# anuunchin/learned-quantization

Hardware: AMD Instinct MI355X
Metric: images/sec training with fake-quant layer, CIFAR-10 bs=256, 1/2/4/8 MI355X (higher is better)
Workload: dtype f32; 1 GPU; fake-quant fwd+bwd (split) on conv-activation batch 256x3x224x224 fp32 per GPU, per_channel scales, lambda=1e-11; per_gpu_batch=256, global_batch=256, parallelism=dp1, buffer_sets=4, launch=eager

## Files before the change

learned_quantization_amd/csrc/lq_kernels.hip:

```cpp
#include <hip/hip_runtime.h>
#include <hip/hip_ext.h>
#include <stdarg.h>
#include <stdlib.h>
#include <stdint.h>
#include <stdio.h>
#include <string.h>

#include <new>
#include <algorithm>
#include <vector>

#include "lq_hip.h"

#include "lq_batch.hpp"
#include "lq_stream2.hpp"
#include "lq_pack.hpp"

namespace lq {

enum Mode { MODE_ROW_BIG = 0, MODE_ROW_SMALL = 1, MODE_COL = 2 };

constexpr int64_t kColRbFused = 48;
constexpr int64_t kColRbBwd = 128;

// ... 519 lines not shown
#undef LQ_PIPE
        return check_hip("pipelined column launch") ? -1 : 1;
        }
    }
    if constexpr (OP == OP_FWD) {
        return 0;
    } else {
        bool seg = false;
        if (pl.L >= 5 && pl.L <= 64 && pl.L % 4 != 0) {
            const int nw = (int)(pl.L + 6) / 4;
            int tl = 1;
            while ((1 << tl) < nw) ++tl;
            const double eff = (double)nw / (double)(1 << tl);
            seg = eff < (OP == OP_FUSED ? 0.8 : 0.7);
        }
        if (!(off & 16384) && seg && pl.R < 4294967296ll) {
            constexpr int kSegU = 2;
            const int rpb = (kBlock * kSegU * 4 - 3) / (int)pl.L;
            const int64_t blocks = ceil_div(pl.R, (int64_t)rpb);
            if (blocks <= 2147483647ll) {
                const FastDiv fL = make_fastdiv((uint32_t)pl.L), fG = make_fastdiv((uint32_t)p.G);
                if (nt) hipLaunchKernelGGL((k_row_seg<OP, 1, kSegU>), dim3((unsigned)blocks), dim3(kBlock), 0, st, p, fL, fG, pl.R, (int)pl.L, rpb, n);
                else hipLaunchKernelGGL((k_row_seg<OP, 0, kSegU>), dim3((unsigned)blocks), dim3(kBlock), 0, st, p, fL, fG, pl.R, (int)pl.L, rpb, n);
                return check_hip("row-segment launch") ? -1 : 1;
            }
        }
        LQ_KNOB(win_all, "LQ_TUNE_WIN", 1);
        if (!(off & 128) && pl.L >= 5 && pl.R < 4294967296ll && (pl.L % 4 != 0 || (win_all && pl.L > 64))) {
            const int nwin = (int)(pl.L % 4 ? (pl.L + 3 + 3) / 4 : pl.L / 4);
            int lg = 1;
            while ((1 << lg) < nwin && lg < 6) ++lg;
            int V = lg == 6 ? (nwin + 63) / 64 : 1;
            if constexpr (OP == OP_BWD) {
                if (nwin >= 17 && nwin <= 32) { lg = 4; V = 2; }
                else if (nwin >= 33 && nwin <= 48) { lg = 4; V = 3; }
                else if (nwin >= 49 && nwin <= 55) { lg = 5; V = 2; }
                else if (nwin >= 65 && nwin <= 84) { lg = 5; V = 3; }
            } else {
                if (nwin >= 17 && nwin <= 32 && (nwin <= 19 || pl.L % 16 == 0)) { lg = 4; V = 2; }
                else if (nwin >= 33 && nwin <= 64) { lg = 5; V = 2; }
            }
            const int U = V == 1 ? 2 : 1;
            const int64_t rows_per_block = (int64_t)kWavesPerBlock * (64 >> lg) * U;
            const int64_t blocks = ceil_div(pl.R, rows_per_block);
            if (blocks <= 2147483647ll && V <= 5) {
                const FastDiv fG = make_fastdiv((uint32_t)p.G);
#define LQ_WIN(NT_, LG_, V_, U_) hipLaunchKernelGGL((k_row_win<OP, NT_, LG_, V_, U_>), dim3((unsigned)blocks), dim3(kBlock), 0, st, p, fG, pl.R, (int)pl.L, n)
#define LQ_WIN2(NT_) do { \
                switch (lg * 8 + V) { \
                    case 1 * 8 + 1: LQ_WIN(NT_, 1, 1, 2); break; \
                    case 2 * 8 + 1: LQ_WIN(NT_, 2, 1, 2); break; \
                    case 3 * 8 + 1: LQ_WIN(NT_, 3, 1, 2); break; \
                    case 4 * 8 + 1: LQ_WIN(NT_, 4, 1, 2); break; \
                    case 4 * 8 + 2: LQ_WIN(NT_, 4, 2, 1); break; \
                    case 4 * 8 + 3: if constexpr (OP == OP_BWD || kDevKnobs) LQ_WIN(NT_, 4, 3, 1); break; \
                    case 5 * 8 + 1: if constexpr (OP != OP_BWD || kDevKnobs) LQ_WIN(NT_, 5, 1, 2); break; \
                    case 5 * 8 + 2: LQ_WIN(NT_, 5, 2, 1); break; \
                    case 5 * 8 + 3: if constexpr (OP == OP_BWD || kDevKnobs) LQ_WIN(NT_, 5, 3, 1); break; \
                    case 6 * 8 + 1: if constexpr (OP == OP_BWD || kDevKnobs) LQ_WIN(NT_, 6, 1, 2); break; \
                    case 6 * 8 + 2: LQ_WIN(NT_, 6, 2, 1); break; \
                    case 6 * 8 + 3: LQ_WIN(NT_, 6, 3, 1); break; \
                    case 6 * 8 + 4: LQ_WIN(NT_, 6, 4, 1); break; \
                    default: LQ_WIN(NT_, 6, 5, 1); break; \
                } } while (0)
#ifdef LQ_DEV_KNOBS
                LQ_KNOB(geom, "LQ_TUNE_WIN_GEOM", 0);
                if (geom >= 100 && nt && ((geom / 10) % 10) * (1 << (geom / 100)) >= nwin) {
                    const int glg = geom / 100, gu = geom % 10;
                    const int64_t gblocks = ceil_div(pl.R, (int64_t)kWavesPerBlock * (64 >> glg) * gu);
                    bool done = true;
#define LQ_WING(LG_, V_, U_) hipLaunchKernelGGL((k_row_win<OP, 1, LG_, V_, U_>), dim3((unsigned)gblocks), dim3(kBlock), 0, st, p, fG, pl.R, (int)pl.L, n)
                    switch (geom) {
                        case 421: LQ_WING(4, 2, 1); break;
                        case 422: LQ_WING(4, 2, 2); break;
                        case 431: LQ_WING(4, 3, 1); break;
                        case 432: LQ_WING(4, 3, 2); break;
                        case 521: LQ_WING(5, 2, 1); break;
                        case 522: LQ_WING(5, 2, 2); break;
                        case 531: LQ_WING(5, 3, 1); break;
                        case 532: LQ_WING(5, 3, 2); break;
                        case 541: LQ_WING(5, 4, 1); break;
                        case 414: LQ_WING(4, 1, 4); break;
                        case 514: LQ_WING(5, 1, 4); break;
                        default: done = false;
                    }
#undef LQ_WING
                    if (done) return check_hip("row-window launch") ? -1 : 1;
                }
#endif
                if (nt) LQ_WIN2(1); else LQ_WIN2(0);
#undef LQ_WIN2
#undef LQ_WIN
                return check_hip("row-window launch") ? -1 : 1;
            }
        }
        if ((off & 8) || pl.L > 64 || pl.L < 8 || pl.L % 4 != 0) return 0;
        const int lg = row_small_lpr_log2_vec(pl.L);
        LQ_KNOB(tiny_u, "LQ_TUNE_TINY_U", 2);
        int U = (1 << lg) < tiny_u ? (1 << lg) : tiny_u;
        if (U != 2 && U != 4) U = 2;
        const int64_t rows_per_block = (int64_t)kWavesPerBlock * (64 >> lg) * U;
        const int64_t blocks = ceil_div(pl.R, rows_per_block);
        if (blocks > 2147483647ll) return 0;
        if (pl.R >= 4294967296ll) return 0;
        const int gm = (p.outer == 1) ? 0 : 1;
#define LQ_TINY3(NT_, U_, LG_) do { \
            if (gm == 0) hipLaunchKernelGGL((k_row_tiny<OP, NT_, U_, LG_, 0>), dim3((unsigned)blocks), dim3(kBlock), 0, st, p, pl.R, (int)pl.L); \
            else hipLaunchKernelGGL((k_row_tiny<OP, NT_, U_, LG_, 1>), dim3((unsigned)blocks), dim3(kBlock), 0, st, p, pl.R, (int)pl.L); } while (0)
#ifdef LQ_DEV_KNOBS
#define LQ_TINY2(NT_) do { \
            if (lg == 1) LQ_TINY3(NT_, 2, 1); \
            else if (lg == 2) { if (U == 2) LQ_TINY3(NT_, 2, 2); else LQ_TINY3(NT_, 4, 2); } \
            else if (lg == 3) { if (U == 2) LQ_TINY3(NT_, 2, 3); else LQ_TINY3(NT_, 4, 3); } \
            else { if (U == 2) LQ_TINY3(NT_, 2, 4); else LQ_TINY3(NT_, 4, 4); } } while (0)
#else
#define LQ_TINY2(NT_) do { \
            if (lg == 1) LQ_TINY3(NT_, 2, 1); \
            else if (lg == 2) LQ_TINY3(NT_, 2, 2); \
            else if (lg == 3) LQ_TINY3(NT_, 2, 3); \
            else LQ_TINY3(NT_, 2, 4); } while (0)
#endif
        if (nt) LQ_TINY2(1); else LQ_TINY2(0);
#undef LQ_TINY2
#undef LQ_TINY3
        return check_hip("tiny-row launch") ? -1 : 1;
    }
}

template <int OP>
constexpr bool kStreamOp = OP == OP_FWD || OP == OP_BWD || OP == OP_FUSED;

template <int OP>
static int launch_traverse(Plan& pl, const Params& p, hipStream_t st) {
    using O = OpT<OP>;
    if (!kStreamOp<OP> && pl.mode == MODE_ROW_BIG && pl.bs != kBlock) return fail(LQ_EINVAL, "internal: operation %d planned with %d-thread units", OP, pl.bs);
    {
        const int r2 = launch_stream2<OP>(pl, p, st);
        if (r2 < 0) return LQ_EHIP;
        if (r2 > 0) return LQ_OK;
    }
    if (pl.mode == MODE_ROW_BIG) {
        const bool vec = aligned(p.P, 16) && (!O::kDy || aligned(p.dy, 16)) && (!O::kStore || aligned(p.out, 16));
        LQ_KNOB(tune_chunk, "LQ_TUNE_CHUNK", 1);
        LQ_KNOB(forced_bs, "LQ_TUNE_BS", 0);
        if (pl.bs == 512 && vec && tune_chunk && !p.direct && !forced_bs && pl.np_ws >= pl.R * row_chunks(pl.L, 1024)) {
            auto fill = [&](int64_t CH) { return (double)pl.L / (double)(row_chunks(pl.L, CH) * CH); };
            const bool k2_form = (OP == OP_BWD || (OP == OP_FUSED && p.tmode >= 1)) && (double)pl.R * (double)pl.L * 4.0 >= (double)kNtBytes;
            const bool small = k2_form ? (row_chunks(pl.L, 4096) > 1 && fill(1024) > fill(4096) + 0.1) : (fill(1024) > fill(2048) + 0.05);
            if (small) {
                pl.bs = 256;
                pl.CH = 1024;
                pl.nc = row_chunks(pl.L, 1024);
                pl.np = pl.R * pl.nc;
                pl.gstride = pl.nc;
                pl.stride1 = p.G * pl.nc;
                pl.n2 = pl.nc;
            }
        }
        const int64_t units = pl.R * pl.nc;
        if (units > 2147483647ll) return fail(LQ_EINVAL, "too many work units (%lld)", (long long)units);
        const int64_t outer_f = pl.R / p.G;
        const int grid3d = (p.G <= 65535 && outer_f <= 65535 && pl.R == outer_f * p.G) ? 1 : 0;
        const dim3 grid = grid3d ? dim3((unsigned)pl.nc, (unsigned)p.G, (unsigned)outer_f) : dim3((unsigned)units);
        const bool nt = kStreamOp<OP> && vec && (double)pl.R * (double)pl.L * 4.0 >= (double)kNtBytes;
        LQ_KNOB(tune_u2, "LQ_TUNE_U2", -1);
        const bool want_u2 = tune_u2 >= 0 ? tune_u2 == 1 : (OP == OP_BWD || p.tmode >= 1);
        const bool u2 = (OP == OP_BWD || OP == OP_FUSED) && want_u2 && vec && nt && pl.bs == 512;
        auto needs_tail = [&](int64_t CH) {
            const int64_t r = pl.L % CH;
            return pl.L % 4 != 0 || (pl.L > CH && r != 0 && r * 8 <= CH);
        };
        if constexpr (OP == OP_BWD || OP == OP_FUSED) if (u2) {
            const int64_t nc2 = row_chunks(pl.L, (int64_t)pl.bs * 8);
            const dim3 grid2 = grid3d ? dim3((unsigned)nc2, (unsigned)p.G, (unsigned)outer_f) : dim3((unsigned)(pl.R * nc2));
            int64_t keep_from = OP == OP_BWD ? mall_keep_from(pl.R * pl.L) : 0;
#ifdef LQ_DEV_KNOBS
            if (g_dev_flags_host & 0x1000) keep_from = -1 - keep_from;
#endif
            if (needs_tail((int64_t)pl.bs * 8))
                hipExtLaunchKernelGGL((k_row_stream<OP, 4, 512, 1, 2, 1>), grid2, dim3(512), 0, st, g_prof_start, g_prof_stop, 0, p, pl.L, nc2, grid3d, keep_from);
            else
                hipExtLaunchKernelGGL((k_row_stream<OP, 4, 512, 1, 2, 0>), grid2, dim3(512), 0, st, g_prof_start, g_prof_stop, 0, p, pl.L, nc2, grid3d, keep_from);
            pl.CH = pl.bs * 8;
            pl.nc = nc2;
            pl.np = pl.R * nc2;
            pl.gstride = nc2;
            pl.stride1 = p.G * nc2;
            pl.n2 = nc2;
            return check_hip("traversal launch");
        }
        const bool tail1 = needs_tail((int64_t)pl.CH);
#define LQ_LAUNCH_STREAM(VEC_, BS_, NT_) do { \
        constexpr bool kTail0 = kDevKnobs || (VEC_ == 4 && !(OP == OP_FWD && (BS_ != kBlock || NT_ != 0)) && !(OP == OP_BWD && BS_ == 512 && NT_ == 1)); \
        constexpr bool kTail1 = kDevKnobs || !(OP == OP_BWD && VEC_ == 4 && BS_ == 512 && NT_ == 1); \
        if (VEC_ == 1 || tail1) { if constexpr (kTail1) hipExtLaunchKernelGGL((k_row_stream<OP, VEC_, BS_, NT_, 1, 1>), grid, dim3(BS_), 0, st, g_prof_start, g_prof_stop, 0, p, pl.L, pl.nc, grid3d, (int64_t)0); } \
        else { if constexpr (kTail0) hipExtLaunchKernelGGL((k_row_stream<OP, VEC_, BS_, NT_, 1, 0>), grid, dim3(BS_), 0, st, g_prof_start, g_prof_stop, 0, p, pl.L, pl.nc, grid3d, (int64_t)0); } } while (0)
        if constexpr (!kStreamOp<OP>) {
            if (vec) LQ_LAUNCH_STREAM(4, 256, 0);
            else LQ_LAUNCH_STREAM(1, 256, 0);
        } else if (!kDevKnobs && OP == OP_FWD && vec && !tail1 && (pl.bs != kBlock || nt)) {
            return fail(LQ_EINVAL, "internal: streaming-size forward of aligned rows reached the row stream");
        } else if (!kDevKnobs && OP == OP_BWD && vec && nt && pl.bs == 512) {
            return fail(LQ_EINVAL, "internal: streaming-size scale gradient reached the one-float4 row stream");
        } else if (vec) {
#ifdef LQ_DEV_KNOBS
            if (pl.bs == 1024) {
                if (nt) LQ_LAUNCH_STREAM(4, 1024, 1);
                else LQ_LAUNCH_STREAM(4, 1024, 0);
            } else
#endif
            if (pl.bs == 512) {
                if (nt) LQ_LAUNCH_STREAM(4, 512, 1);
                else LQ_LAUNCH_STREAM(4, 512, 0);
            } else {
                if (nt) LQ_LAUNCH_STREAM(4, 256, 1);
                else LQ_LAUNCH_STREAM(4, 256, 0);
            }
        } else {
#ifdef LQ_DEV_KNOBS
            if (pl.bs == 1024) LQ_LAUNCH_STREAM(1, 1024, 0);
            else
#endif
            if (pl.bs == 512) LQ_LAUNCH_STREAM(1, 512, 0);
            else LQ_LAUNCH_STREAM(1, 256, 0);
        }
#undef LQ_LAUNCH_STREAM
    } else if (pl.mode == MODE_ROW_SMALL) {
        const bool vec = row_small_vec(pl, p.P, O::kDy ? p.dy : nullptr, O::kStore ? p.out : nullptr);
        const int lg = vec ? row_small_lpr_log2_vec(pl.L) : pl.lpr_log2;
        const int64_t blocks = ceil_div(pl.R, kBlock >> lg);
        if (blocks > 2147483647ll) return fail(LQ_EINVAL, "too many blocks (%lld)", (long long)blocks);
        if (vec) hipLaunchKernelGGL((k_row_small<OP, 4>), dim3((unsigned)blocks), dim3(kBlock), 0, st, p, pl.R, (int)pl.L, lg);
        else hipLaunchKernelGGL((k_row_small<OP, 1>), dim3((unsigned)blocks), dim3(kBlock), 0, st, p, pl.R, (int)pl.L, lg);
    } else {
        int variant;
        int64_t nbx;
        col_variant(pl, p.P, O::kDy ? p.dy : nullptr, O::kStore ? p.out : nullptr, variant, nbx);
        const int64_t blocks = nbx * pl.ysplit;
        if (blocks > 2147483647ll) return fail(LQ_EINVAL, "too many blocks (%lld)", (long long)blocks);
        hipLaunchKernelGGL((k_col<OP>), dim3((unsigned)blocks), dim3(kBlock), 0, st, p, pl.C, pl.rps, nbx, variant, pl.ysplit);
    }
    return check_hip("traversal launch");
}

static bool finalize_cols_single(const FinGeom& f) {
    return finalize_cols_ok(f.groups, f.gstride, f.n1, f.stride1, f.n2) && f.n1 <= 64 && f.n1 * f.groups * f.n2 >= 131072;
}

template <int OP, bool COLS = true>
static int launch_finalize(const Params& p, FinGeom f, hipStream_t st) {
    const int form = finalize_form(f.groups, f.n1, f.stride1, f.n2);
    if (COLS && finalize_cols_single(f)) {
        if constexpr (COLS) hipLaunchKernelGGL((k_finalize_cols<OP>), dim3((unsigned)ceil_div(f.groups, 64 / f.n2)), dim3(kBlock), 0, st, p, f);
    } else if (form == 0) {
        hipLaunchKernelGGL((k_finalize_thread<OP>), dim3((unsigned)ceil_div(f.groups, kBlock)), dim3(kBlock), 0, st, p, f);
    } else if (form == 1) {
        hipLaunchKernelGGL((k_finalize_block<OP, 64>), dim3((unsigned)f.groups), dim3(64), 0, st, p, f);
    } else if (form == 2) {
        hipLaunchKernelGGL((k_finalize_block<OP, 256>), dim3((unsigned)f.groups), dim3(256), 0, st, p, f);
    } else {
        hipLaunchKernelGGL((k_finalize_block<OP, 1024>), dim3((unsigned)f.groups), dim3(1024), 0, st, p, f);
    }
    return check_hip("finalize launch");
}

static FinGeom group_geom(const Plan& pl, int64_t outer, int64_t G, int64_t inner) {
    FinGeom f;
    memset(&f, 0, sizeof(f));
    f.groups = G;
    f.gstride = pl.gstride;
    f.n1 = pl.n1;
    f.stride1 = pl.stride1;
    f.n2 = pl.n2;
    f.count = (double)outer * (double)inner;
    return f;
}

static FinGeom global_geom(const Plan& pl, int64_t outer, int64_t G, int64_t inner) {
    FinGeom f;
    memset(&f, 0, sizeof(f));
    f.groups = 1;
    f.gstride = 0;
    f.n1 = 1;
    f.stride1 = 0;
    f.n2 = pl.np;
    f.count = (double)outer * (double)G * (double)inner;
    return f;
}

static Params base_params(const float* P, const float* s, int64_t outer, int64_t G, int64_t inner) {
    Params p;
    memset(&p, 0, sizeof(p));
    p.P = P;
    p.s = s;
    p.outer = outer;
    p.G = G;
    p.inner = inner;
    return p;
}

static bool make_conv_tile(ConvTile& ct, int64_t hw, int64_t ci, int64_t co, int64_t outer, int64_t G, int64_t inner);
static int64_t conv_tile_partials(const ConvTile& ct, int64_t G);
static void conv_tile_fin(const ConvTile& ct, int64_t G, int64_t& gstride, int64_t& n1, int64_t& stride1, int64_t& n2);

}

using namespace lq;

#define LQ_REQUIRE_PTR(x)                                                      \
    do {                                                                       \
        if (!(x)) return fail(LQ_EINVAL, "%s: argument '%s' is NULL", __func__, #x); \
        if (!aligned((x), 4)) return fail(LQ_EALIGN, "%s: argument '%s' is not 4-byte aligned", __func__, #x); \
    } while (0)

extern "C" {

int lq_version(void) { return LQ_ABI_VERSION; }

#ifdef LQ_DEV_KNOBS
int lq_dev_set_ablate(int mask) {
    return hipMemcpyToSymbol(HIP_SYMBOL(lq::g_ablate), &mask, sizeof(int)) == hipSuccess ? LQ_OK : LQ_EHIP;
}
#endif

#ifdef LQ_DEV_KNOBS
int lq_dev_set_flags(int bits) {
    g_dev_flags_host = bits;
    return hipMemcpyToSymbol(HIP_SYMBOL(lq::g_dev_flags), &bits, sizeof(int)) == hipSuccess ? LQ_OK : LQ_EHIP;
}
#endif

#ifdef LQ_DEV_KNOBS
int lq_dev_set_trace(void* buf) {
    unsigned long long* b = (unsigned long long*)buf;
    return hipMemcpyToSymbol(HIP_SYMBOL(lq::g_trace), &b, sizeof(b)) == hipSuccess ? LQ_OK : LQ_EHIP;
}
#endif

int lq_profile_events(void* start, void* stop) {
    g_prof_start = (hipEvent_t)start;
    g_prof_stop = (hipEvent_t)stop;
    return LQ_OK;
}

const char* lq_last_error(void) { return g_err; }

const char* lq_status_string(int status) {
    switch (status) {
        case LQ_OK: return "LQ_OK";
        case LQ_EINVAL: return "LQ_EINVAL";
        case LQ_EHIP: return "LQ_EHIP";
        case LQ_EWORKSPACE: return "LQ_EWORKSPACE";
        case LQ_EALIGN: return "LQ_EALIGN";
        default: return "LQ_UNKNOWN";
    }
}

size_t lq_workspace_bytes(int64_t outer, int64_t G, int64_t inner) {
    if (outer <= 0 || G <= 0 || inner <= 0) return 0;
    return ws_bytes_for(make_plan(outer, G, inner));
}

int lq_fq_forward(const float* P, const float* s, float* out, void* q, int q_dtype, int64_t outer, int64_t G,
                  int64_t inner, void* stream) {
    int rc = check_desc(outer, G, inner);
    if (rc) return rc;
    LQ_REQUIRE_PTR(P);
    LQ_REQUIRE_PTR(s);
    if (!out && !q) return fail(LQ_EINVAL, "lq_fq_forward: both out and q are NULL");
    if (q_dtype < LQ_Q_NONE || q_dtype > LQ_Q_I8) return fail(LQ_EINVAL, "lq_fq_forward: bad q_dtype %d", q_dtype);
    if ((q != nullptr) != (q_dtype != LQ_Q_NONE)) return fail(LQ_EINVAL, "lq_fq_forward: q and q_dtype disagree");
    Plan pl = make_plan(outer, G, inner);
    Params p = base_params(P, s, outer, G, inner);
    p.q = q;
    p.q_dtype = q_dtype;
    if (out) {
        if (!aligned(out, 4)) return fail(LQ_EALIGN, "lq_fq_forward: out is not 4-byte aligned");
        p.out = out;
        return launch_traverse<OP_FWD>(pl, p, (hipStream_t)stream);
    }
    pl = make_plan(outer, G, inner, kBlock);
    return launch_traverse<OP_QONLY>(pl, p, (hipStream_t)stream);
}

static int check_conv(const char* fn, int64_t hw, int64_t ci, int64_t co, int64_t outer, int64_t G, int64_t inner) {
    if (hw <= 0 || ci <= 0 || co <= 0) return fail(LQ_EINVAL, "%s: hw, ci, co must be positive", fn);
    const double n = (double)hw * (double)ci * (double)co;
    if (n != (double)outer * (double)G * (double)inner) return fail(LQ_EINVAL, "%s: hw*ci*co does not match the tensor", fn);
    if (n >= 4294967296.0) return fail(LQ_EINVAL, "%s: conv kernels must have fewer than 2^32 elements", fn);
    return LQ_OK;
}

int lq_fq_forward_oihw(const float* P, const float* s, float* out, float* out_oihw, int64_t hw, int64_t ci, int64_t co,
                       int64_t outer, int64_t G, int64_t inner, void* stream) {
    int rc = check_desc(outer, G, inner);
    if (rc) return rc;
    if ((rc = check_conv("lq_fq_forward_oihw", hw, ci, co, outer, G, inner))) return rc;
    LQ_REQUIRE_PTR(P);
    LQ_REQUIRE_PTR(s);
    LQ_REQUIRE_PTR(out_oihw);
    if (!out && !(aligned(P, 16) && lq_conv_tile_supported(hw, ci, co, outer, G, inner)))
        return fail(LQ_EINVAL, "lq_fq_forward_oihw: out may be NULL only for kernels the LDS-tile path takes (lq_conv_tile_supported) with P 16-byte aligned");
    Plan pl = make_plan(outer, G, inner, kBlock);
    Params p = base_params(P, s, outer, G, inner);
    p.out = out;
    p.out_perm = out_oihw;
    p.perm_hw = (uint32_t)hw;
    p.perm_ci = (uint32_t)ci;
    p.perm_co = (uint32_t)co;
    ConvTile ct;
    if (aligned(P, 16) && aligned(out, 16) && make_conv_tile(ct, hw, ci, co, outer, G, inner)) {
        hipLaunchKernelGGL(k_conv_tile_fwd, dim3(ct.ntc * ct.nto), dim3(kBlock), 0, (hipStream_t)stream, p, ct);
        return check_hip("conv tile forward launch");
    }
// ... 1247 lines not shown
```

learned_quantization_amd/csrc/lq_traverse.hpp:

```cpp
#ifndef LQ_TRAVERSE_HPP_
#define LQ_TRAVERSE_HPP_
#include "lq_reduce.hpp"

namespace lq {

typedef float v4f __attribute__((ext_vector_type(4)));

template <int NT>
__device__ __forceinline__ float4 load4(const float* p) {
    if (NT) {
        const v4f v = __builtin_nontemporal_load(reinterpret_cast<const v4f*>(p));
        return make_float4(v.x, v.y, v.z, v.w);
    }
    return *reinterpret_cast<const float4*>(p);
}
template <int NT>
__device__ __forceinline__ void store4(float* p, const float4& v) {
    if (NT) {
        const v4f t = {v.x, v.y, v.z, v.w};
        __builtin_nontemporal_store(t, reinterpret_cast<v4f*>(p));
    } else {
        *reinterpret_cast<float4*>(p) = v;
    }
}

__device__ __forceinline__ void store4_sc1nt(float* p, const float4& v) {
    const v4f t = {v.x, v.y, v.z, v.w};
    asm volatile("global_store_dwordx4 %0, %1, off sc1 nt" : : "v"(p), "v"(t) : "memory");
}
#ifdef LQ_DEV_KNOBS
__device__ __forceinline__ void store4_policy(int pol, float* p, const float4& v) {
    const v4f t = {v.x, v.y, v.z, v.w};
    if (pol == 1) asm volatile("global_store_dwordx4 %0, %1, off" : : "v"(p), "v"(t) : "memory");
    else if (pol == 2) asm volatile("global_store_dwordx4 %0, %1, off sc1 nt" : : "v"(p), "v"(t) : "memory");
    else if (pol == 3) asm volatile("global_store_dwordx4 %0, %1, off sc0 sc1 nt" : : "v"(p), "v"(t) : "memory");
    else if (pol == 4) asm volatile("global_store_dwordx4 %0, %1, off sc1" : : "v"(p), "v"(t) : "memory");
    else if (pol == 5) asm volatile("global_store_dwordx4 %0, %1, off sc0 sc1" : : "v"(p), "v"(t) : "memory");
    else __builtin_nontemporal_store(t, reinterpret_cast<v4f*>(p));
}
#endif

typedef float v4f_u __attribute__((ext_vector_type(4), aligned(4)));
__device__ __forceinline__ float4 load4_keep(const float* p) {
    asm volatile("; default-policy load" : : : );
    const v4f_u v = *reinterpret_cast<const v4f_u*>(p);
    asm volatile("; end" : : : );
    return make_float4(v.x, v.y, v.z, v.w);
}

template <int NT, int UA>
__device__ __forceinline__ float4 load4x(const float* p) {
    if (!UA) return load4<NT>(p);
    const v4f_u v = NT ? __builtin_nontemporal_load(reinterpret_cast<const v4f_u*>(p)) : *reinterpret_cast<const v4f_u*>(p);
    return make_float4(v.x, v.y, v.z, v.w);
}
template <int NT, int UA>
__device__ __forceinline__ void store4x(float* p, const float4& v) {
    if (!UA) {
        store4<NT>(p, v);
        return;
    }
    const v4f_u t = {v.x, v.y, v.z, v.w};
    if (NT) __builtin_nontemporal_store(t, reinterpret_cast<v4f_u*>(p));
    else *reinterpret_cast<v4f_u*>(p) = t;
}

template <int OP, int VEC, int NT, int U>
constexpr bool kMallWalk = OP == OP_BWD && VEC == 4 && NT == 1 && U == 2;

template <int OP, int VEC, int BS, int NT, int U = 1, int TAIL = 1>
__device__ __forceinline__ void row_stream_body(const Params& p, int64_t L, int64_t nc, int64_t row, int64_t ck, int64_t g,
                                                int64_t keep_from = 0) {
    using O = OpT<OP>;
    constexpr int CH = BS * 4 * U;
    const int64_t base = row * L + ck * (int64_t)CH;
    [[maybe_unused]] const bool keep = kMallWalk<OP, VEC, NT, U> && base >= keep_from;
    const int64_t rem = L - ck * (int64_t)CH;
    const int len = (ck == nc - 1) ? (int)rem : CH;
    Acc acc = O::template init<Acc>();

    if (VEC == 4) {
        const int phase = (int)(base & 3);
        int head = (4 - phase) & 3;
        if (head > len) head = len;
        const int64_t vbase = base + head;
        const int vlen = len - head;
        const int len4 = vlen >> 2;
        int64_t i[U];
        float4 x[U], d[U];
#pragma unroll
        for (int u = 0; u < U; ++u) {
            const int j = u * BS + (int)threadIdx.x;
            i[u] = vbase + (int64_t)(j < len4 ? j : 0) * 4;
            const int64_t il = len4 > 0 ? i[u] : vbase - 4;
            if (kMallWalk<OP, VEC, NT, U> && keep) x[u] = load4_keep(p.P + il);
            else x[u] = load4<NT>(p.P + il);
            d[u] = x[u];
            if (O::kDy) d[u] = load4<NT>(p.dy + il);
        }
        const bool fold = TAIL && len4 > BS * U;
        const int je = BS * U + (int)threadIdx.x;
        float4 xe = make_float4(0.f, 0.f, 0.f, 0.f), de = xe;
        if (__builtin_expect(fold && je < len4, 0)) {
            const int64_t ie0 = vbase + (int64_t)je * 4;
            xe = load4<NT>(p.P + ie0);
            de = xe;
            if (O::kDy) de = load4<NT>(p.dy + ie0);
        }
        const int tail = vlen & 3;
        const int t = (int)threadIdx.x;
        const bool edge = TAIL && (t < head || (t >= 8 && t - 8 < tail));
        const int64_t is = t < head ? base + t : vbase + (int64_t)len4 * 4 + (t - 8);
        float xs = 0.f, dsc = 0.f;
        if (edge) {
            xs = p.P[is];
            if (O::kDy) dsc = p.dy[is];
        }
        __builtin_amdgcn_sched_barrier(0);
        const Ctx ctx = O::ctx(p, g);
#pragma unroll
        for (int u = 0; u < U; ++u) {
            const int j = u * BS + (int)threadIdx.x;
            if (j < len4) {
                float4 r;
                if constexpr (O::kVec4) {
                    r = O::elem4(p, ctx, i[u], x[u], d[u], acc);
                } else {
                    r.x = O::elem(p, ctx, i[u] + 0, x[u].x, O::kDy ? d[u].x : 0.f, acc);
                    r.y = O::elem(p, ctx, i[u] + 1, x[u].y, O::kDy ? d[u].y : 0.f, acc);
                    r.z = O::elem(p, ctx, i[u] + 2, x[u].z, O::kDy ? d[u].z : 0.f, acc);
                    r.w = O::elem(p, ctx, i[u] + 3, x[u].w, O::kDy ? d[u].w : 0.f, acc);
                }
                if (O::kStore) store4<NT>(p.out + i[u], r);
            }
        }
        if (__builtin_expect(fold, 0)) {
            if (je < len4) {
                const int64_t ie = vbase + (int64_t)je * 4;
                float4 r;
                if constexpr (O::kVec4) {
                    r = O::elem4(p, ctx, ie, xe, de, acc);
                } else {
                    r.x = O::elem(p, ctx, ie + 0, xe.x, O::kDy ? de.x : 0.f, acc);
                    r.y = O::elem(p, ctx, ie + 1, xe.y, O::kDy ? de.y : 0.f, acc);
                    r.z = O::elem(p, ctx, ie + 2, xe.z, O::kDy ? de.z : 0.f, acc);
                    r.w = O::elem(p, ctx, ie + 3, xe.w, O::kDy ? de.w : 0.f, acc);
                }
                if (O::kStore) store4<NT>(p.out + ie, r);
            }
        }
        if (edge) {
            float r = O::elem(p, ctx, is, xs, dsc, acc);
            if (O::kStore) p.out[is] = r;
        }
    } else {
        float x[4 * U], d[4 * U];
#pragma unroll
        for (int u = 0; u < 4 * U; ++u) {
            const int j = u * BS + (int)threadIdx.x;
            const int jc = j < len ? j : len - 1;
            x[u] = p.P[base + jc];
            d[u] = O::kDy ? p.dy[base + jc] : 0.f;
        }
        const Ctx ctx = O::ctx(p, g);
#pragma unroll
        for (int u = 0; u < 4 * U; ++u) {
            const int j = u * BS + (int)threadIdx.x;
            if (j < len) {
                float r = O::elem(p, ctx, base + j, x[u], d[u], acc);
                if (O::kStore) p.out[base + j] = r;
            }
        }
        for (int j = 4 * U * BS + (int)threadIdx.x; j < len; j += BS) {
            float r = O::elem(p, ctx, base + j, p.P[base + j], O::kDy ? p.dy[base + j] : 0.f, acc);
            if (O::kStore) p.out[base + j] = r;
        }
    }
    if (O::kReduce) {
        [[maybe_unused]] Acc acc2;
        if constexpr (O::kSecond) acc2 = O::take_second(acc);
        if constexpr (O::kStdMerge) {
            block_reduce_dpp<BS>(acc);
        } else {
            block_reduce<O, Acc, BS>(acc);
        }
        if (threadIdx.x == 0) write_partial_t<OP>(p, row * nc + ck, acc);
        if constexpr (O::kSecond) {
            __syncthreads();
            block_reduce_dpp<BS>(acc2);
            if (threadIdx.x == 0) write_partial_second(p, row * nc + ck, acc2);
        }
    }
}

template <int OP, int VEC, int BS, int NT, int U = 1, int TAIL = 1>
__global__ __launch_bounds__(BS, (BS == 1024 ? 8 : 0)) void k_row_stream(Params p, int64_t L, int64_t nc, int grid3d, int64_t keep_from) {
    constexpr bool kRev = kMallWalk<OP, VEC, NT, U>;
#ifdef LQ_DEV_KNOBS
    const bool rev = kRev && keep_from >= 0;
    if (kRev && !rev) keep_from = -1 - keep_from;
#else
    constexpr bool rev = kRev;
#endif
    int64_t row, ck, g;
    if (grid3d) {
        ck = rev ? gridDim.x - 1 - blockIdx.x : blockIdx.x;
        g = rev ? gridDim.y - 1 - blockIdx.y : blockIdx.y;
        row = (int64_t)(rev ? gridDim.z - 1 - blockIdx.z : blockIdx.z) * p.G + g;
    } else {
        const int64_t unit = rev ? gridDim.x - 1 - blockIdx.x : blockIdx.x;
        row = unit / nc;
        ck = unit - row * nc;
        g = row % p.G;
    }
    row_stream_body<OP, VEC, BS, NT, U, TAIL>(p, L, nc, row, ck, g, keep_from);
}

template <int OP, int VEC>
__device__ __forceinline__ void row_small_body(const Params& p, int64_t R, int L, int lpr_log2, int64_t blk) {
    using O = OpT<OP>;
    const int lpr = 1 << lpr_log2;
    const int team = (int)threadIdx.x >> lpr_log2;
    const int lane = (int)threadIdx.x & (lpr - 1);
    const int64_t row = blk * (kBlock >> lpr_log2) + team;
    const bool valid = row < R;
    Acc acc = O::template init<Acc>();
    if (valid) {
        const Ctx ctx = O::ctx(p, row % p.G);
        const int64_t base = row * (int64_t)L;
        if (VEC == 4) {
            const int L4 = L >> 2;
#pragma unroll 2
            for (int j = lane; j < L4; j += lpr) {
                const int64_t i = base + (int64_t)j * 4;
                const float4 x = *reinterpret_cast<const float4*>(p.P + i);
                float4 d = x;
                if (O::kDy) d = *reinterpret_cast<const float4*>(p.dy + i);
                float4 r;
                if constexpr (O::kVec4) {
                    r = O::elem4(p, ctx, i, x, d, acc);
                } else {
                    r.x = O::elem(p, ctx, i + 0, x.x, O::kDy ? d.x : 0.f, acc);
                    r.y = O::elem(p, ctx, i + 1, x.y, O::kDy ? d.y : 0.f, acc);
                    r.z = O::elem(p, ctx, i + 2, x.z, O::kDy ? d.z : 0.f, acc);
                    r.w = O::elem(p, ctx, i + 3, x.w, O::kDy ? d.w : 0.f, acc);
                }
                if (O::kStore) *reinterpret_cast<float4*>(p.out + i) = r;
            }
        } else {
#pragma unroll 4
            for (int j = lane; j < L; j += lpr) {
                const float x = p.P[base + j];
                const float d = O::kDy ? p.dy[base + j] : 0.f;
                float r = O::elem(p, ctx, base + j, x, d, acc);
                if (O::kStore) p.out[base + j] = r;
            }
        }
    }
    if (O::kReduce) {
        [[maybe_unused]] Acc acc2;
        if constexpr (O::kSecond) {
            acc2 = O::take_second(acc);
            wave_reduce<O>(acc2, lpr);
        }
        wave_reduce<O>(acc, lpr);
        if (valid && lane == 0) {
            const int64_t o = row / p.G, g = row - o * p.G;
            write_partial_t<OP>(p, (p.G > 1 ? g * p.outer + o : row), acc);
            if constexpr (O::kSecond) write_partial_second(p, (p.G > 1 ? g * p.outer + o : row), acc2);
        }
    }
}

template <int OP, int VEC>
__global__ __launch_bounds__(kBlock) void k_row_small(Params p, int64_t R, int L, int lpr_log2) {
    row_small_body<OP, VEC>(p, R, L, lpr_log2, (int64_t)blockIdx.x);
}

constexpr int kColUnroll = 4;

template <class O>
__device__ __forceinline__ void col_cross_wave(Acc* lds, const Acc& mine, int slot, int slots) {
    lds[(threadIdx.x >> 6) * slots + slot] = mine;
}

template <int OP, int VW, int NT>
__device__ __forceinline__ void col_tile_body(const Params& p, int64_t C, int64_t RB, int64_t bx, int64_t by, Acc* lds) {
    using O = OpT<OP>;
    const int lane = threadIdx.x & 63, w = threadIdx.x >> 6;
    const int64_t col0 = (bx * 64 + lane) * VW;
    const bool active = col0 < C;
    Ctx ctx[VW];
    Acc acc[VW];
#pragma unroll
    for (int k = 0; k < VW; ++k) {
        acc[k] = O::template init<Acc>();
        ctx[k] = O::ctx(p, active ? (col0 + k) / p.inner : 0);
    }
    const int64_t r0 = by * RB;
    const int64_t r1 = (r0 + RB < p.outer) ? r0 + RB : p.outer;
    if (active) {
        for (int64_t r = r0 + w; r < r1; r += 4 * kColUnroll) {
            float x[kColUnroll][VW], d[kColUnroll][VW];
#pragma unroll
            for (int u = 0; u < kColUnroll; ++u) {
                const int64_t rr = (r + 4 * u < r1) ? r + 4 * u : r1 - 1;
                const int64_t i = rr * C + col0;
                if (VW == 4) {
                    const float4 v = load4<NT>(p.P + i);
                    x[u][0] = v.x; x[u][1 % VW] = v.y; x[u][2 % VW] = v.z; x[u][3 % VW] = v.w;
                    if (O::kDy) {
                        const float4 e = load4<NT>(p.dy + i);
                        d[u][0] = e.x; d[u][1 % VW] = e.y; d[u][2 % VW] = e.z; d[u][3 % VW] = e.w;
                    }
                } else {
                    x[u][0] = p.P[i];
                    if (O::kDy) d[u][0] = p.dy[i];
                }
            }
#pragma unroll
            for (int u = 0; u < kColUnroll; ++u) {
                if (r + 4 * u < r1) {
                    const int64_t i = (r + 4 * u) * C + col0;
                    if constexpr (VW == 4 && O::kVec4c) {
                        const float4 xv = make_float4(x[u][0], x[u][1 % VW], x[u][2 % VW], x[u][3 % VW]);
                        const float4 dv = O::kDy ? make_float4(d[u][0], d[u][1 % VW], d[u][2 % VW], d[u][3 % VW]) : xv;
                        const float4 ov = O::elem4c(p, ctx, i, xv, dv, acc);
                        if (O::kStore) store4<NT>(p.out + i, ov);
                    } else {
                        float o[VW];
#pragma unroll
                        for (int k = 0; k < VW; ++k) o[k] = O::elem(p, ctx[k], i + k, x[u][k], O::kDy ? d[u][k] : 0.f, acc[k]);
                        if (O::kStore) {
                            if (VW == 4) store4<NT>(p.out + i, make_float4(o[0], o[1 % VW], o[2 % VW], o[3 % VW]));
                            else p.out[i] = o[0];
                        }
                    }
                }
            }
        }
    }
    if (O::kReduce) {
        [[maybe_unused]] Acc acc2[VW];
        if constexpr (O::kSecond) {
#pragma unroll
            for (int k = 0; k < VW; ++k) acc2[k] = O::take_second(acc[k]);
        }
#pragma unroll
        for (int k = 0; k < VW; ++k) lds[w * (64 * VW) + lane * VW + k] = acc[k];
        __syncthreads();
        if (w == 0 && active) {
#pragma unroll
            for (int k = 0; k < VW; ++k) {
                Acc r = lds[lane * VW + k];
#pragma unroll
                for (int ww = 1; ww < 4; ++ww) O::merge(r, lds[ww * (64 * VW) + lane * VW + k]);
                write_partial_t<OP>(p, by * C + col0 + k, r);
            }
        }
        if constexpr (O::kSecond) {
            __syncthreads();
#pragma unroll
            for (int k = 0; k < VW; ++k) lds[w * (64 * VW) + lane * VW + k] = acc2[k];
            __syncthreads();
            if (w == 0 && active) {
#pragma unroll
                for (int k = 0; k < VW; ++k) {
                    Acc r = lds[lane * VW + k];
// ... 131 lines not shown
            Acc r = O::template init<Acc>();
            for (int e = e0 + h * C; e < kBlock * 4; e += H * C) O::merge(r, lds[e]);
            lds2[h * C + c] = r;
        }
        __syncthreads();
        if ((int)threadIdx.x < C) {
            Acc r = lds2[threadIdx.x];
            for (int hh = 1; hh < H; ++hh) O::merge(r, lds2[hh * C + (int)threadIdx.x]);
            write_partial_t<OP>(p, blk * C + threadIdx.x, r);
        }
    }
}

constexpr int kColLdsAcc = kBlock * 5;
template <int OP, bool P4 = true>
__device__ __forceinline__ void col_body(const Params& p, int64_t C, int64_t RB, int64_t nbx, int variant, int64_t b, int64_t nby, Acc* lds) {
    if (variant == 0) {
        col_small_body<OP>(p, (int)C, RB, b, lds);
    } else if (P4 && variant == 6) {
        if constexpr (P4) col_periodic4_body<OP, 0>(p, (int)C, nby, b, lds);
    } else if (P4 && variant == 7) {
        if constexpr (P4) col_periodic4_body<OP, 1>(p, (int)C, nby, b, lds);
    } else {
        const int64_t by = b / nbx, bx = b - by * nbx;
        if (variant == 5) col_tile_body<OP, 4, 1>(p, C, RB, bx, by, lds);
        else if (variant == 4) col_tile_body<OP, 4, 0>(p, C, RB, bx, by, lds);
        else col_tile_body<OP, 1, 0>(p, C, RB, bx, by, lds);
    }
}

template <int OP>
__global__ __launch_bounds__(kBlock) void k_col(Params p, int64_t C, int64_t RB, int64_t nbx, int variant, int64_t nby) {
    __shared__ Acc lds[OpT<OP>::kReduce ? kColLdsAcc : 1];
    col_body<OP>(p, C, RB, nbx, variant, (int64_t)blockIdx.x, nby, lds);
}

struct FinGeom {
    int64_t groups;
    int64_t gstride, n1, stride1, n2;
    double count;
    float* o0;
    float* o1;
    uint32_t* o2;
    int accum;
};

template <int OP>
struct FinT;

template <>
struct FinT<OP_BWD> {
    __device__ static float emit(const Params& p, const FinGeom& f, int64_t g, const AccW& a) {
        const float maxq = __uint_as_float(a.a);
        float mean;
        if (a.b == 0.0) {
            mean = -1.0f * fabsf(tanhf(p.lam));
        } else {
            mean = (float)(a.c / f.count);
        }
        const float ds = mean * maxq;
        f.o0[g] = ds;
        if (f.o1) {
            f.o1[g] = maxq;
            f.o1[f.groups + g] = mean;
            f.o1[2 * f.groups + g] = (float)a.b;
        }
        return ds;
    }
};
template <>
struct FinT<OP_FUSED> : FinT<OP_BWD> {};
template <>
struct FinT<OP_BWD_PERM> : FinT<OP_BWD> {};

template <>
struct FinT<OP_MAXBIN_FWD> {
    __device__ static float emit(const Params&, const FinGeom& f, int64_t g, const AccW& a) {
        f.o0[g] = __uint_as_float(a.a);
        f.o2[g] = (uint32_t)(a.b > 4294967295.0 ? 4294967295.0 : a.b);
        return 0.f;
    }
};

template <>
struct FinT<OP_DIFF_FWD> {
    __device__ static float emit(const Params&, const FinGeom& f, int64_t g, const AccW& a) {
        f.o0[g] = (float)(a.c / f.count);
        return 0.f;
    }
};

template <>
struct FinT<OP_DIFF_BWD> {
    __device__ static float emit(const Params&, const FinGeom& f, int64_t g, const AccW& a) {
        const float v = (float)a.c;
        f.o0[g] = f.accum ? f.o0[g] + v : v;
        return 0.f;
    }
};
template <>
struct FinT<OP_DIFF_BWD_V> : FinT<OP_DIFF_BWD> {};

template <>
struct FinT<OP_STE_SCALE> {
    __device__ static float emit(const Params& p, const FinGeom& f, int64_t g, const AccW& a) {
        const float ds = (float)((double)p.c_scale * a.c);
        f.o0[g] = ds;
        return ds;
    }
};

template <int OP>
__device__ __forceinline__ void emit_direct(const Params& p, int64_t g, const Acc& acc) {
    FinGeom f;
    f.groups = p.G;
    f.gstride = f.n1 = f.stride1 = f.n2 = 0;
    f.count = p.ecount;
    f.o0 = p.e0;
    f.o1 = p.e1;
    f.o2 = nullptr;
    f.accum = 0;
    AccW w;
    w.a = acc.a;
    w.b = (double)acc.b;
    w.c = acc.c;
    FinT<OP>::emit(p, f, g, w);
}

template <class O>
__device__ __forceinline__ AccW load_partial(const Params& p, int64_t idx) {
    AccW w;
    w.a = p.pa[idx];
    w.b = (double)p.pb[idx];
    w.c = p.pc[idx];
    return w;
}

template <int CTRL, int ROW_MASK>
__device__ __forceinline__ void dpp_step_w(AccW& acc) {
    const uint32_t a = dpp_u32<CTRL, ROW_MASK>(0u, acc.a);
    const double b = dpp_f64<CTRL, ROW_MASK>(acc.b);
    const double c = dpp_f64<CTRL, ROW_MASK>(acc.c);
    acc.a = a > acc.a ? a : acc.a;
    acc.b += b;
    acc.c += c;
}
__device__ __forceinline__ void dpp_row_reduce_w(AccW& acc) {
    dpp_step_w<0xB1, 0xf>(acc);
    dpp_step_w<0x4E, 0xf>(acc);
    dpp_step_w<0x141, 0xf>(acc);
    dpp_step_w<0x140, 0xf>(acc);
}

template <int OP, int BS>
__device__ __forceinline__ float finalize_block_body(const Params& p, const FinGeom& f, int64_t g, int tid) {
    float ret = 0.f;
    using O = OpT<OP>;
    const int64_t n = f.n1 * f.n2;
    const int64_t gbase = g * f.gstride;
    AccW acc = O::template init<AccW>();
    if (n < 0x7fffffffll) {
        const uint32_t n32 = (uint32_t)n, n2 = (uint32_t)f.n2;
        for (uint32_t k = (uint32_t)tid; k < n32; k += BS) {
            const uint32_t i1 = k / n2, i2 = k - i1 * n2;
            O::merge(acc, load_partial<O>(p, gbase + (int64_t)i1 * f.stride1 + i2));
        }
    } else {
        for (int64_t k = tid; k < n; k += BS) {
            const int64_t i1 = k / f.n2, i2 = k - i1 * f.n2;
            O::merge(acc, load_partial<O>(p, gbase + i1 * f.stride1 + i2));
        }
    }
    if constexpr (O::kStdMerge) {
        constexpr int NW = BS / 64;
        __shared__ uint32_t sa[NW];
        __shared__ double sb[NW], sc[NW];
        dpp_row_reduce_w(acc);
        dpp_step_w<0x142, 0xa>(acc);
        dpp_step_w<0x143, 0xc>(acc);
        const int lane = tid & 63, wid = tid >> 6;
        if (NW > 1) {
            if (lane == 63) {
                sa[wid] = acc.a;
                sb[wid] = acc.b;
                sc[wid] = acc.c;
            }
            __syncthreads();
            if (wid == 0) {
                AccW r;
                r.a = lane < NW ? sa[lane] : 0u;
                r.b = lane < NW ? sb[lane] : 0.0;
                r.c = lane < NW ? sc[lane] : 0.0;
                dpp_row_reduce_w(r);
                if (lane == 0) ret = FinT<OP>::emit(p, f, g, r);
            }
        } else if (lane == 63) {
            ret = FinT<OP>::emit(p, f, g, acc);
        }
    } else {
        block_reduce<O, AccW, BS>(acc);
        if (tid == 0) ret = FinT<OP>::emit(p, f, g, acc);
    }
    return ret;
}

template <int OP, int BS>
__global__ __launch_bounds__(BS) void k_finalize_block(Params p, FinGeom f) {
    finalize_block_body<OP, BS>(p, f, (int64_t)blockIdx.x, (int)threadIdx.x);
}

template <int OP>
__device__ __forceinline__ float finalize_thread_body(const Params& p, const FinGeom& f, int64_t g) {
    using O = OpT<OP>;
    AccW acc = O::template init<AccW>();
    for (int64_t i1 = 0; i1 < f.n1; ++i1)
        for (int64_t i2 = 0; i2 < f.n2; ++i2) O::merge(acc, load_partial<O>(p, g * f.gstride + i1 * f.stride1 + i2));
    return FinT<OP>::emit(p, f, g, acc);
}

__host__ __device__ inline int finalize_form(int64_t groups, int64_t n1, int64_t stride1, int64_t n2) {
    const int64_t n = n1 * n2;
    if (n <= 4 || (n <= 32 && groups >= 2048)) return 0;
    (void)stride1;
    return n <= 256 ? 1 : (n <= 1024 ? 2 : 3);
}

__host__ __device__ inline bool finalize_cols_ok(int64_t groups, int64_t gstride, int64_t n1, int64_t stride1, int64_t n2) {
    return n1 > 1 && n2 >= 1 && n2 <= 64 && gstride == n2 && stride1 == groups * n2 && groups * n2 >= 64;
}

template <int OP, int AH>
__device__ __forceinline__ void finalize_cols_walk(const Params& p, int64_t col, int64_t C, int64_t n1, int wv, AccW& acc) {
    using O = OpT<OP>;
    for (int64_t i = wv; i < n1; i += 4 * AH) {
        AccW v[AH];
#pragma unroll
        for (int u = 0; u < AH; ++u) v[u] = load_partial<O>(p, col + (i + 4 * u < n1 ? i + 4 * u : i) * C);
#pragma unroll
        for (int u = 0; u < AH; ++u)
            if (i + 4 * u < n1) O::merge(acc, v[u]);
    }
}

template <int OP>
__device__ __forceinline__ bool finalize_cols_body(const Params& p, const FinGeom& f, int64_t g0, AccW* lds, int64_t& g, AccW& acc) {
    using O = OpT<OP>;
    const int inner = (int)f.n2, gpb = 64 / inner;
    const int lane = threadIdx.x & 63, wv = threadIdx.x >> 6;
    const int64_t col = g0 * inner + lane, C = f.stride1, n1 = f.n1;
    acc = O::template init<AccW>();
    if (lane < gpb * inner && col < C) {
        if (n1 <= 32) finalize_cols_walk<OP, 8>(p, col, C, n1, wv, acc);
        else finalize_cols_walk<OP, 16>(p, col, C, n1, wv, acc);
    }
    lds[threadIdx.x] = acc;
    __syncthreads();
    g = g0 + threadIdx.x;
    const bool emits = (int)threadIdx.x < gpb && g < f.groups;
    if (emits) {
        acc = O::template init<AccW>();
        for (int k = 0; k < inner; ++k)
            for (int ww = 0; ww < 4; ++ww) O::merge(acc, lds[ww * 64 + threadIdx.x * inner + k]);
    }
    return emits;
}

template <int OP>
__global__ __launch_bounds__(kBlock) void k_finalize_cols(Params p, FinGeom f) {
    __shared__ AccW lds[kBlock];
    int64_t g;
    AccW acc;
    if (finalize_cols_body<OP>(p, f, (int64_t)blockIdx.x * (64 / (int)f.n2), lds, g, acc)) FinT<OP>::emit(p, f, g, acc);
}

template <int OP>
__global__ __launch_bounds__(kBlock) void k_finalize_thread(Params p, FinGeom f) {
    const int64_t g = (int64_t)blockIdx.x * kBlock + threadIdx.x;
    if (g >= f.groups) return;
    finalize_thread_body<OP>(p, f, g);
}

}

#endif
```

Before: 2.714 million images/s.

## Store row-stream partials group-major and gather contiguous runs in finalize

Row-stream kernels now write per-block partial reductions in a group-major layout, so all partials belonging to one channel group are contiguous. When that layout holds, the block finalize kernel switches to a run gather that reads a flat contiguous range with several loads issued ahead, instead of doing strided div/mod index arithmetic. The goal is coalesced, latency-hidden partial loads in the finalize step. Cost: extra kernel arguments, a new invariant that rows are whole layers of groups (now enforced with an error), and a runtime branch inside the finalize kernel.

```diff
diff --git a/learned_quantization_amd/csrc/lq_kernels.hip b/learned_quantization_amd/csrc/lq_kernels.hip
--- a/learned_quantization_amd/csrc/lq_kernels.hip
+++ b/learned_quantization_amd/csrc/lq_kernels.hip
@@ -695,14 +695,25 @@
                 pl.CH = 1024;
                 pl.nc = row_chunks(pl.L, 1024);
                 pl.np = pl.R * pl.nc;
-                pl.gstride = pl.nc;
-                pl.stride1 = p.G * pl.nc;
-                pl.n2 = pl.nc;
             }
         }
         const int64_t units = pl.R * pl.nc;
         if (units > 2147483647ll) return fail(LQ_EINVAL, "too many work units (%lld)", (long long)units);
         const int64_t outer_f = pl.R / p.G;
+        if (pl.R != outer_f * p.G) return fail(LQ_EINVAL, "internal: %lld rows are not whole layers of %lld groups", (long long)pl.R, (long long)p.G);
+        bool group_major = OP != OP_DIFF_FWD;
+#ifdef LQ_DEV_KNOBS
+        if (g_dev_flags_host & 0x2000) group_major = false;
+#endif
+        int64_t ps_g = 0, ps_o = 0;
+        auto set_partials = [&](int64_t nc) {
+            ps_g = group_major ? outer_f * nc : nc;
+            ps_o = group_major ? nc : p.G * nc;
+            pl.gstride = ps_g;
+            pl.stride1 = ps_o;
+            pl.n2 = nc;
+        };
+        set_partials(pl.nc);
         const int grid3d = (p.G <= 65535 && outer_f <= 65535 && pl.R == outer_f * p.G) ? 1 : 0;
         const dim3 grid = grid3d ? dim3((unsigned)pl.nc, (unsigned)p.G, (unsigned)outer_f) : dim3((unsigned)units);
         const bool nt = kStreamOp<OP> && vec && (double)pl.R * (double)pl.L * 4.0 >= (double)kNtBytes;
@@ -720,24 +731,22 @@
 #ifdef LQ_DEV_KNOBS
             if (g_dev_flags_host & 0x1000) keep_from = -1 - keep_from;
 #endif
+            set_partials(nc2);
             if (needs_tail((int64_t)pl.bs * 8))
-                hipExtLaunchKernelGGL((k_row_stream<OP, 4, 512, 1, 2, 1>), grid2, dim3(512), 0, st, g_prof_start, g_prof_stop, 0, p, pl.L, nc2, grid3d, keep_from);
+                hipExtLaunchKernelGGL((k_row_stream<OP, 4, 512, 1, 2, 1>), grid2, dim3(512), 0, st, g_prof_start, g_prof_stop, 0, p, pl.L, nc2, grid3d, keep_from, ps_g, ps_o);
             else
-                hipExtLaunchKernelGGL((k_row_stream<OP, 4, 512, 1, 2, 0>), grid2, dim3(512), 0, st, g_prof_start, g_prof_stop, 0, p, pl.L, nc2, grid3d, keep_from);
+                hipExtLaunchKernelGGL((k_row_stream<OP, 4, 512, 1, 2, 0>), grid2, dim3(512), 0, st, g_prof_start, g_prof_stop, 0, p, pl.L, nc2, grid3d, keep_from, ps_g, ps_o);
             pl.CH = pl.bs * 8;
             pl.nc = nc2;
             pl.np = pl.R * nc2;
-            pl.gstride = nc2;
-            pl.stride1 = p.G * nc2;
-            pl.n2 = nc2;
             return check_hip("traversal launch");
         }
         const bool tail1 = needs_tail((int64_t)pl.CH);
 #define LQ_LAUNCH_STREAM(VEC_, BS_, NT_) do { \
         constexpr bool kTail0 = kDevKnobs || (VEC_ == 4 && !(OP == OP_FWD && (BS_ != kBlock || NT_ != 0)) && !(OP == OP_BWD && BS_ == 512 && NT_ == 1)); \
         constexpr bool kTail1 = kDevKnobs || !(OP == OP_BWD && VEC_ == 4 && BS_ == 512 && NT_ == 1); \
-        if (VEC_ == 1 || tail1) { if constexpr (kTail1) hipExtLaunchKernelGGL((k_row_stream<OP, VEC_, BS_, NT_, 1, 1>), grid, dim3(BS_), 0, st, g_prof_start, g_prof_stop, 0, p, pl.L, pl.nc, grid3d, (int64_t)0); } \
-        else { if constexpr (kTail0) hipExtLaunchKernelGGL((k_row_stream<OP, VEC_, BS_, NT_, 1, 0>), grid, dim3(BS_), 0, st, g_prof_start, g_prof_stop, 0, p, pl.L, pl.nc, grid3d, (int64_t)0); } } while (0)
+        if (VEC_ == 1 || tail1) { if constexpr (kTail1) hipExtLaunchKernelGGL((k_row_stream<OP, VEC_, BS_, NT_, 1, 1>), grid, dim3(BS_), 0, st, g_prof_start, g_prof_stop, 0, p, pl.L, pl.nc, grid3d, (int64_t)0, ps_g, ps_o); } \
+        else { if constexpr (kTail0) hipExtLaunchKernelGGL((k_row_stream<OP, VEC_, BS_, NT_, 1, 0>), grid, dim3(BS_), 0, st, g_prof_start, g_prof_stop, 0, p, pl.L, pl.nc, grid3d, (int64_t)0, ps_g, ps_o); } } while (0)
         if constexpr (!kStreamOp<OP>) {
             if (vec) LQ_LAUNCH_STREAM(4, 256, 0);
             else LQ_LAUNCH_STREAM(1, 256, 0);
@@ -793,16 +802,27 @@
 template <int OP, bool COLS = true>
 static int launch_finalize(const Params& p, FinGeom f, hipStream_t st) {
     const int form = finalize_form(f.groups, f.n1, f.stride1, f.n2);
+    int run = finalize_run_ok(f.gstride, f.n1, f.stride1, f.n2) ? 1 : 0;
+#ifdef LQ_DEV_KNOBS
+    if (g_dev_flags_host & 0x2000) run = 0;
+    const int force = (g_dev_flags_host >> 14) & 3;
+    if (force && form >= 1 && !(COLS && finalize_cols_single(f))) {
+        if (force == 1) hipLaunchKernelGGL((k_finalize_block<OP, 256>), dim3((unsigned)f.groups), dim3(256), 0, st, p, f, run);
+        else if (force == 2) hipLaunchKernelGGL((k_finalize_block<OP, 512>), dim3((unsigned)f.groups), dim3(512), 0, st, p, f, run);
+        else hipLaunchKernelGGL((k_finalize_block<OP, 1024>), dim3((unsigned)f.groups), dim3(1024), 0, st, p, f, run);
+        return check_hip("finalize launch");
+    }
+#endif
     if (COLS && finalize_cols_single(f)) {
         if constexpr (COLS) hipLaunchKernelGGL((k_finalize_cols<OP>), dim3((unsigned)ceil_div(f.groups, 64 / f.n2)), dim3(kBlock), 0, st, p, f);
     } else if (form == 0) {
         hipLaunchKernelGGL((k_finalize_thread<OP>), dim3((unsigned)ceil_div(f.groups, kBlock)), dim3(kBlock), 0, st, p, f);
     } else if (form == 1) {
-        hipLaunchKernelGGL((k_finalize_block<OP, 64>), dim3((unsigned)f.groups), dim3(64), 0, st, p, f);
+        hipLaunchKernelGGL((k_finalize_block<OP, 64>), dim3((unsigned)f.groups), dim3(64), 0, st, p, f, run);
     } else if (form == 2) {
-        hipLaunchKernelGGL((k_finalize_block<OP, 256>), dim3((unsigned)f.groups), dim3(256), 0, st, p, f);
+        hipLaunchKernelGGL((k_finalize_block<OP, 256>), dim3((unsigned)f.groups), dim3(256), 0, st, p, f, run);
     } else {
-        hipLaunchKernelGGL((k_finalize_block<OP, 1024>), dim3((unsigned)f.groups), dim3(1024), 0, st, p, f);
+        hipLaunchKernelGGL((k_finalize_block<OP, 1024>), dim3((unsigned)f.groups), dim3(1024), 0, st, p, f, run);
     }
     return check_hip("finalize launch");
 }
diff --git a/learned_quantization_amd/csrc/lq_traverse.hpp b/learned_quantization_amd/csrc/lq_traverse.hpp
--- a/learned_quantization_amd/csrc/lq_traverse.hpp
+++ b/learned_quantization_amd/csrc/lq_traverse.hpp
@@ -70,7 +70,7 @@
 
 template <int OP, int VEC, int BS, int NT, int U = 1, int TAIL = 1>
 __device__ __forceinline__ void row_stream_body(const Params& p, int64_t L, int64_t nc, int64_t row, int64_t ck, int64_t g,
-                                                int64_t keep_from = 0) {
+                                                int64_t keep_from = 0, int64_t pi = -1) {
     using O = OpT<OP>;
     constexpr int CH = BS * 4 * U;
     const int64_t base = row * L + ck * (int64_t)CH;
@@ -184,17 +184,18 @@
         } else {
             block_reduce<O, Acc, BS>(acc);
         }
-        if (threadIdx.x == 0) write_partial_t<OP>(p, row * nc + ck, acc);
+        if (threadIdx.x == 0) write_partial_t<OP>(p, pi < 0 ? row * nc + ck : pi, acc);
         if constexpr (O::kSecond) {
             __syncthreads();
             block_reduce_dpp<BS>(acc2);
-            if (threadIdx.x == 0) write_partial_second(p, row * nc + ck, acc2);
+            if (threadIdx.x == 0) write_partial_second(p, pi < 0 ? row * nc + ck : pi, acc2);
         }
     }
 }
 
 template <int OP, int VEC, int BS, int NT, int U = 1, int TAIL = 1>
-__global__ __launch_bounds__(BS, (BS == 1024 ? 8 : 0)) void k_row_stream(Params p, int64_t L, int64_t nc, int grid3d, int64_t keep_from) {
+__global__ __launch_bounds__(BS, (BS == 1024 ? 8 : 0)) void k_row_stream(Params p, int64_t L, int64_t nc, int grid3d, int64_t keep_from,
+                                                                        int64_t pstride_g, int64_t pstride_o) {
     constexpr bool kRev = kMallWalk<OP, VEC, NT, U>;
 #ifdef LQ_DEV_KNOBS
     const bool rev = kRev && keep_from >= 0;
@@ -202,18 +203,20 @@
 #else
     constexpr bool rev = kRev;
 #endif
-    int64_t row, ck, g;
+    int64_t row, ck, g, o;
     if (grid3d) {
         ck = rev ? gridDim.x - 1 - blockIdx.x : blockIdx.x;
         g = rev ? gridDim.y - 1 - blockIdx.y : blockIdx.y;
-        row = (int64_t)(rev ? gridDim.z - 1 - blockIdx.z : blockIdx.z) * p.G + g;
+        o = rev ? gridDim.z - 1 - blockIdx.z : blockIdx.z;
+        row = o * p.G + g;
     } else {
         const int64_t unit = rev ? gridDim.x - 1 - blockIdx.x : blockIdx.x;
         row = unit / nc;
         ck = unit - row * nc;
-        g = row % p.G;
-    }
-    row_stream_body<OP, VEC, BS, NT, U, TAIL>(p, L, nc, row, ck, g, keep_from);
+        o = row / p.G;
+        g = row - o * p.G;
+    }
+    row_stream_body<OP, VEC, BS, NT, U, TAIL>(p, L, nc, row, ck, g, keep_from, g * pstride_g + o * pstride_o + ck);
 }
 
 template <int OP, int VEC>
@@ -651,14 +654,39 @@
     dpp_step_w<0x140, 0xf>(acc);
 }
 
+__host__ __device__ inline bool finalize_run_ok(int64_t gstride, int64_t n1, int64_t stride1, int64_t n2) {
+    return n1 == 1 || (stride1 == n2 && gstride == n1 * n2);
+}
+constexpr int kRunAhead = 4;
+
 template <int OP, int BS>
+__device__ __forceinline__ void finalize_run_gather(const Params& p, int64_t gbase, int64_t n, int tid, AccW& acc) {
+    using O = OpT<OP>;
+    for (int64_t k0 = tid; k0 < n; k0 += (int64_t)kRunAhead * BS) {
+        AccW v[kRunAhead];
+#pragma unroll
+        for (int u = 0; u < kRunAhead; ++u) {
+            const int64_t k = k0 + (int64_t)u * BS;
+            v[u] = load_partial<O>(p, gbase + (k < n ? k : n - 1));
+        }
+#pragma unroll
+        for (int u = 0; u < kRunAhead; ++u) asm volatile("" : "+v"(v[u].a), "+v"(v[u].b), "+v"(v[u].c));
+#pragma unroll
+        for (int u = 0; u < kRunAhead; ++u)
+            if (k0 + (int64_t)u * BS < n) O::merge(acc, v[u]);
+    }
+}
+
+template <int OP, int BS, bool RUN = false>
 __device__ __forceinline__ float finalize_block_body(const Params& p, const FinGeom& f, int64_t g, int tid) {
     float ret = 0.f;
     using O = OpT<OP>;
     const int64_t n = f.n1 * f.n2;
     const int64_t gbase = g * f.gstride;
     AccW acc = O::template init<AccW>();
-    if (n < 0x7fffffffll) {
+    if constexpr (RUN) {
+        finalize_run_gather<OP, BS>(p, gbase, n, tid, acc);
+    } else if (n < 0x7fffffffll) {
         const uint32_t n32 = (uint32_t)n, n2 = (uint32_t)f.n2;
         for (uint32_t k = (uint32_t)tid; k < n32; k += BS) {
             const uint32_t i1 = k / n2, i2 = k - i1 * n2;
@@ -704,8 +732,9 @@
 }
 
 template <int OP, int BS>
-__global__ __launch_bounds__(BS) void k_finalize_block(Params p, FinGeom f) {
-    finalize_block_body<OP, BS>(p, f, (int64_t)blockIdx.x, (int)threadIdx.x);
+__global__ __launch_bounds__(BS) void k_finalize_block(Params p, FinGeom f, int run) {
+    if (run) finalize_block_body<OP, BS, true>(p, f, (int64_t)blockIdx.x, (int)threadIdx.x);
+    else finalize_block_body<OP, BS>(p, f, (int64_t)blockIdx.x, (int)threadIdx.x);
 }
 
 template <int OP>
```

Result: no change. 2.709 million images/s (-0.2%).
